# emiliofidalgo/liodom

Measured on AMD Instinct MI355X. Metric: scans/sec (64×1800 cloud, prev_frames=20) at 1 GPU; pose RMSE vs CPU ref, higher is better.
Workload: dtype f64

## Files before the change

liodom_amd/csrc/handle_plan.h:

```cpp
#pragma once
#include <algorithm>
#include <climits>
#include <cstdio>
#include <cstdlib>
#include <cstring>

#include "../../include/liodom_hip.h"
#include "liodom_sizes.h"

namespace liodom_dev {

struct HandleEnv {
  bool pipe_flags = true;
  bool map_rows = true;
  int hash_build = -1;
  int lds_cells_max = kLdsCellsMax;
  bool early_rebuild = true;
  bool safe_mode = false;
  int debug_clocks = 0;
  bool ring_split = true;
  bool ring_split_lb = true;
  int ring_pitch = 0;
  bool hash_incr = true;
  float rebuild_delta = 0.25f;
// ... 129 lines not shown
      config->n_streams < 1 || config->max_points < 1 || !(params->max_range > params->min_range)) {
    *error = "liodom_create: parameter out of range";
    return LIODOM_ERR_INVALID_ARG;
  }
  return LIODOM_OK;
}

inline int plan_handle(const liodom_params_t* params, const liodom_config_t* config, const HandleCaps& caps, const HandleEnv& env,
                       HandlePlan* out, const char** error) {
  using plan_detail::cdiv;
  using plan_detail::round_up;
  if (int rc = plan_check_params(params, config, error)) return rc;
  HandlePlan p;
  const int S = config->n_streams, H = params->scan_lines, P = (int)params->local_map_size;

  p.min_range = params->min_range; p.max_range = params->max_range;
  p.lidar_type = params->lidar_type; p.scan_lines = H;
  p.scan_regions = params->scan_regions; p.edges_per_region = params->edges_per_region;
  p.min_points_per_scan = (long long)params->min_points_per_scan;
  p.prev_frames = P;
  p.apply_on_ftol = config->lm_apply_step_on_ftol;
  p.rotation_mode = config->pose_rotation_mode != 0 ? 1 : 0;
  p.filter_local_map = (params->filter_local_map && !params->mapping) ? 1 : 0;
  p.vox_inv = 1.0f / 0.4f;
  p.n_streams = S;
  p.max_points = config->max_points;
  p.ring_cap = config->max_points;
  p.use_imu = params->use_imu ? 1 : 0;
  p.mapping = params->mapping ? 1 : 0;
  p.pose_log_cap = std::max(1, config->pose_log_capacity);
  p.pose_covariance = config->pose_covariance != 0;
  p.map_rows = env.map_rows;
  p.lds_cells_max = env.lds_cells_max;
  p.rebuild_delta = env.rebuild_delta;
  p.hb_slack_min = env.hb_slack; p.hb_new_room = env.hb_new_room;
  p.knn_save = env.knn_save;
  p.knn_exact_only = env.knn_exact_only ? 1 : 0;
  p.wait_ticks = (unsigned long long)(env.wait_ms * 1.0e5);
  p.lockstep = S >= 16;

  const long long slots = (long long)params->scan_regions * ((long long)params->edges_per_region + 1);
  if (slots > INT_MAX || ring_extract_lds_bytes((int)slots, params->scan_regions) > 160 * 1024) {
    *error = "pick lists (scan_regions * (edges_per_region + 1)) exceed 160 KiB of LDS";
    return LIODOM_ERR_CAPACITY;
  }
  p.slots_per_ring = (int)slots;
  p.ring_lds_bytes = ring_extract_lds_bytes(p.slots_per_ring, params->scan_regions);
  const int edges = H * p.slots_per_ring;
  p.edge_cap = (int)round_up(std::max(1, edges), 64);
  if (lm_lds_bytes(p.edge_cap) + 16384 > 160 * 1024) {
    *error = "liodom_create: edge capacity too large for the solve's LDS tile";
    return LIODOM_ERR_INVALID_ARG;
  }

  p.lds_hash_build = env.hash_build < 0 ? p.lockstep : env.hash_build != 0;

  p.use_flags = !p.lockstep && !env.serialised && env.pipe_flags;
  p.flag_gate = !(S == 1 && cdiv(cdiv(p.edge_cap, 8), 2) * 4 <= (long long)caps.cus * 12);

  {
    const int auto_g = S > 4 ? 1 : (edges >= 2048 ? kLmGroupsMax : (edges >= 512 ? 4 : 1));
    p.lm_groups = config->lm_workgroups == 0 ? auto_g : std::max(1, std::min(kLmGroupsMax, config->lm_workgroups));
  }

  p.early_rebuild = (!p.lds_hash_build && !p.filter_local_map && !params->mapping && S <= 4 && env.early_rebuild) ? 1 : 0;

  if (env.safe_mode) plan_enter_safe_mode(&p);

  p.recv_cap = p.mapping ? (config->recv_capacity > 0 ? config->recv_capacity : 262144) : 0;
  const long long map_cap = (long long)p.edge_cap * P + p.recv_cap;
  const long long pad = p.early_rebuild ? 8LL * p.edge_cap : 0;
  long long ts = 1024;
  while (ts < 2 * (map_cap + pad)) ts <<= 1;
  if (p.lds_hash_build && ts < kLdsSlots) ts = kLdsSlots;
  const long long used_cap = map_cap + pad;
  const long long ovf_base = map_cap + pad;
  long long sorted_cap = p.early_rebuild ? ovf_base + p.edge_cap : map_cap;
  const bool incr_sized = env.hash_incr && p.lockstep && p.lds_hash_build && !params->mapping && !params->filter_local_map && !p.early_rebuild;
  if (incr_sized) sorted_cap = 2 * map_cap + 65536 + (long long)(kHbPeriod - 1) * p.edge_cap;

  p.debug = config->debug_buffers & 1;
  if (caps.instrumented && env.debug_clocks != 0) {
    const int dc = env.debug_clocks;
    p.debug |= ((dc & (128 | 256)) ? (dc & 32) : 32) | (dc & (64 | 128)) | (dc & ~255);
  }
  const long long ring_id_stride = round_up((long long)config->max_points + 512, 256);
  p.tile_cap = (int)std::max(1LL, cdiv(config->max_points, kTilePts));
  p.split_pad = (int)round_up(p.tile_cap, 8);
  p.lb_hpad = (int)round_up(H, 64);
  p.ring_split_lb = p.lockstep && params->lidar_type == 0 && !p.safe_mode && env.ring_split_lb;
  const long long ring_pitch = env.ring_pitch ? env.ring_pitch : round_up(cdiv((long long)config->max_points * 9, (long long)H * 8), 8);

  if (ts > (1LL << 30) || map_cap > INT_MAX || used_cap > INT_MAX || sorted_cap > INT_MAX || ring_id_stride > INT_MAX || ring_pitch > INT_MAX) {
    *error = "liodom_create: capacities (window, received map, points per scan) exceed 32-bit sizes";
    return LIODOM_ERR_CAPACITY;
  }
  p.map_cap = (int)map_cap; p.table_size = (int)ts;
  p.used_cap = (int)used_cap; p.ovf_base = (int)ovf_base; p.sorted_cap = (int)sorted_cap;
  p.ring_id_stride = (size_t)ring_id_stride;
  p.ring_pitch = (int)ring_pitch;
  p.ring_stride = p.ring_split_lb ? std::max((size_t)config->max_points, (size_t)H * (size_t)p.ring_pitch) : (size_t)config->max_points;

  p.ring_split = env.ring_split && !p.safe_mode;
  if (p.ring_split) {
    long long budget = (long long)std::max(0, caps.ring_split_wgs_per_cu) * std::max(0, caps.cus) / 2;
    if (budget > 256) budget = 256;
    p.ring_split_max_wgs = (int)budget;
    if (p.tile_cap > p.ring_split_max_wgs) p.ring_split = false;
  }

  p.knn8 = p.lockstep && env.knn8;
  p.knn8_grid = (int)std::max(1LL, cdiv(cdiv(p.edge_cap, kKnn8Queries), kKnnGridDiv));
  p.hash_incr = (env.hash_incr && p.knn8 && p.lds_hash_build && !params->mapping && !params->filter_local_map && P > kHbPeriod &&
                 sorted_cap >= 2 * map_cap + (long long)(kHbPeriod - 1) * p.edge_cap) ? 1 : 0;
  p.hb_spill_base = p.sorted_cap - (kHbPeriod - 1) * p.edge_cap;
  p.knn_queries = p.lockstep ? 4 : 8;
  p.knn_partials = p.lockstep ? 0 : 1;
  p.knn_blocks = (int)round_up(cdiv(p.edge_cap, p.knn_queries), 4);
  p.knn_grid = (int)std::max(1LL, cdiv(p.knn_blocks, kKnnGridDiv));
  p.mask_stride = (int)round_up(p.knn_blocks, 128);

  p.ov_ok = env.knn_overlap != 0 && p.early_rebuild && S == 1 && p.knn_partials &&
            (env.knn_overlap == 2 || (long long)p.knn_grid * 4 * 3 <= (long long)caps.cus * 24);
  p.chain_ok = p.early_rebuild && S == 1 && p.knn_partials && !p.use_imu && (long long)p.knn_grid * 4 * 2 <= (long long)caps.cus * 24 &&
               env.knn_overlap != 0 && env.chain;
  p.speculate = (p.ov_ok || p.chain_ok) ? env.speculate : 0;
  p.spec_backoff = 16;
  p.spec_theta = env.spec_theta;

  *out = p;
  return LIODOM_OK;
}

struct OverlapModes { bool ov, chain; };
inline OverlapModes plan_overlap_modes(const HandlePlan& p, bool alone) {
  const bool base = p.early_rebuild && p.use_flags && alone;
  return {base && p.ov_ok, base && p.chain_ok && !p.flag_gate};
}

struct ModesRuntime {
  bool alone = true;
  bool streams_concurrent = true;
  int hb_stats[4] = {0, 0, 0, 0}, spec_stats[4] = {0, 0, 0, 0};
  unsigned int chain_count = 0, done0 = 0, done1 = 0;
  double replay_enqueue_us = 0.0, replay_wait_us = 0.0;
  int n_lagged = 0, n_readers = 0, n_hits = 0;
  long long subset_steps = 0;
};

inline void plan_format_modes(const HandlePlan& p, const ModesRuntime& r, char* buf, int cap) {
  const OverlapModes om = plan_overlap_modes(p, r.alone);
  snprintf(buf, (size_t)cap,
           "n_streams=%d early_rebuild=%d hash_build=%s pipe_flags=%d flag_gate=%d lm_groups=%d knn_instance=%d knn_queries=%d "
           "knn_grid=%d/%d knn8=%d hash_incr=%d hash_rebuilds=%d hash_appends=%d hash_appends_spilled=%d hash_points_spilled=%d knn_partials=%d knn_saved_bound=%d knn_exact_only=%d line_gate_kernel=%d filter_local_map=%d mapping=%d "
           "rotation_mode=%d table_size=%d sorted_cap=%d hb_spill_base=%d rebuild_delta=%.3f knn_overlap=%d streams_concurrent=%d safe_mode=%d ring_split=%d ring_split_max_wgs=%d ring_split_lb=%d chain=%d speculate=%d spec_early=%d/%d spec_unconfirmed=%d/%d chain_done=%u/%u/%u replay_enqueue_us=%.2f replay_wait_us=%.2f debug=%d",
           p.n_streams, p.early_rebuild, p.early_rebuild ? "streamed" : (p.lds_hash_build ? "lds" : "global"), p.use_flags ? 1 : 0,
           (p.use_flags && p.flag_gate) ? 1 : 0, p.lm_groups, p.lockstep ? 128 : 256, p.knn_queries, p.knn_grid,
           p.knn_blocks, p.knn8 ? 1 : 0, p.hash_incr, r.hb_stats[0], r.hb_stats[1], r.hb_stats[2], r.hb_stats[3], p.knn_partials,
           p.knn_save >= 2 ? 2 : (p.knn_save >= 1 ? 1 : 0), p.knn_exact_only, p.lockstep ? 1 : 0, p.filter_local_map, p.mapping,
           p.rotation_mode, p.table_size, p.sorted_cap, p.hb_spill_base, (double)p.rebuild_delta,
           (om.ov || om.chain) ? 1 : 0, r.streams_concurrent ? 1 : 0, p.safe_mode ? 1 : 0, p.ring_split ? 1 : 0, p.ring_split ? p.ring_split_max_wgs : 0, p.ring_split_lb ? 1 : 0,
           om.chain ? 1 : 0, p.speculate, r.spec_stats[0], r.spec_stats[2], r.spec_stats[1], r.spec_stats[3], r.chain_count, r.done0, r.done1,
           r.replay_enqueue_us, r.replay_wait_us, p.debug);
  auto tail = [&](size_t* room) { const size_t n = std::strlen(buf); *room = (size_t)cap - n; return buf + n; };
  size_t room = 0;
  if (p.pose_covariance) { char* t = tail(&room); snprintf(t, room, " pose_cov=1"); }
  if (r.n_lagged > 0) { char* t = tail(&room); snprintf(t, room, " mapper_lag=%d", r.n_lagged); }
// ... 7 lines not shown
```

liodom_amd/csrc/kernels_lm.h:

```cpp
constexpr int kLmWaves = kLmThreads / 64;


__device__ int lm_compact_bits(const DevView& v, int s, int outer_it, int E, int* idx ) {
  const int lane = threadIdx.x & 63;
  const int Q = v.knn_queries;
  const int nb = (E + Q - 1) / Q;
  const int nwords = (nb + 3) >> 2;
  const unsigned int* mw = reinterpret_cast<const unsigned int*>(v.corr_mask + ((size_t)s * 2 + outer_it) * v.mask_stride);
  int run = 0;
  for (int w0 = 0; w0 < nwords; w0 += 64) {
    const int w = w0 + lane;
    unsigned int word = (w < nwords) ? mw[w] : 0u;
    const int pop = __popc(word);
    const int incl = wave_incl_scan_i32(pop);
    int o = run + incl - pop;
    while (word) {
      const int b = __ffs(word) - 1;
      word &= word - 1u;
      const int bit = w * 32 + b;
      idx[o++] = (bit >> 3) * Q + (bit & 7);
    }
    run += readlane_i32(incl, 63);
  }
  return run;
// ... 238 lines not shown
  if (lane < 24) {
    const unsigned long long bits = (unsigned long long)__double_as_longlong(T[lane >> 1]);
    word = (lane & 1) ? (unsigned int)(bits >> 32) : (unsigned int)bits;
  }
  __hip_atomic_store((gu64*)(base + lane), ((unsigned long long)tag << 32) | word, __ATOMIC_RELAXED, __HIP_MEMORY_SCOPE_AGENT);
}

template <bool kList = false>
__global__ void k_imu_override(DevView v, int s0, int count) {
  const int i = blockIdx.x * blockDim.x + threadIdx.x;
  if (i >= count) return;
  const int s = stream_of_lane<kList>(v, s0, i);
  StreamState& st = v.state[s];
  if (!st.initialized) return;
  double odom[12], out[12], l2b[12], q[4];
#pragma unroll
  for (int k = 0; k < 12; k++) { odom[k] = st.odom[k]; l2b[k] = v.laser_to_base[k]; }
#pragma unroll
  for (int k = 0; k < 4; k++) q[k] = v.imu_q[(size_t)s * 4 + k];
  imu_override(odom, q, l2b, v.rotation_mode, out);
#pragma unroll
  for (int k = 0; k < 12; k++) st.odom[k] = out[k];
  quat_from_pose(out, v.rotation_mode, st.param_q);
  st.param_t[0] = out[3]; st.param_t[1] = out[7]; st.param_t[2] = out[11];
}

__device__ __forceinline__ void pose_cov_store(const DevView& v, int s, const StreamState& st, const LmState& lm, const double* acc, int nblocks, int tid) {
  const int j = tid - 64;
  if (j < 0 || j >= 21) return;
  PoseCovRaw* r = v.cov_raw + s;
  bool applied = lm.termination == LM_TERM_FUNC_TOL && lm.apply_on_ftol != 0;
  for (int k = 0; k < 4; k++) applied = applied && lm.q[k] == lm.cand_q[k];
  for (int k = 0; k < 3; k++) applied = applied && lm.t[k] == lm.cand_t[k];
  r->H[j] = applied ? acc[7 + j] : lm.H[j];
  if (j == 0) {
    r->scan_index = st.info.scan_index; r->n_res = nblocks; r->termination = lm.termination; r->has_solve = 1;
    r->cost = lm.cost;
  }
}

__device__ __forceinline__ void rebuild_beside_solve(const DevView& v, int s, StreamState& st, int eb, int outer_it, int block, int nblocks, unsigned int seq, int* sbase, int* sslot);

template <int kOuterIt, bool kChainMode, bool kList = false>
#ifndef LIODOM_LM_WAVES_PER_SIMD
#define LIODOM_LM_WAVES_PER_SIMD 1
#endif
__global__ __launch_bounds__(kLmThreads, LIODOM_LM_WAVES_PER_SIMD) void k_lm_solve(DevView v, int s0, int eb, unsigned int seq, unsigned int done_target) {
  constexpr int outer_it = kOuterIt;
  constexpr int chain = kChainMode ? 1 : 0;
  __shared__ double sh_pose2[2][12];
  __shared__ int sh_pi, sh_ci;
  __shared__ int sh_nmoved;
  __shared__ double sh_pred_s[20];
  __shared__ int sh_unapplied;
  __shared__ double sh_acc[kAccN];
  __shared__ LmState lm;
  __shared__ int sh_flag;
  __shared__ int sh_C;
  const int s = stream_of<kList>(v, s0, (int)blockIdx.y);
#if defined(LIODOM_CHAIN_PRIO)
  if (v.n_streams <= 4) __builtin_amdgcn_s_setprio(LIODOM_CHAIN_PRIO);
#endif
  const int G = v.lm_groups, gstride = G > 1 ? 8 : 1, bxl = (int)blockIdx.x;
  const bool is_solver = bxl < G * gstride && (bxl % gstride) == 0;
  const int g = is_solver ? bxl / gstride : G + (bxl < G * gstride ? bxl - (bxl / gstride + 1) : bxl - G);
  StreamState& st = v.state[s];
  __shared__ int sh_cnt[kMaxFrames + 1];
  OV_STAMP(v, bxl == 0 && threadIdx.x == 0, outer_it == 0 ? 0 : 3);
  if (seq && outer_it == 0 && bxl == 0 && threadIdx.x == 0) {
    typedef __attribute__((address_space(1))) unsigned int gu32;
    __hip_atomic_store((gu32*)(v.ov_flags + s), seq, __ATOMIC_RELAXED, __HIP_MEMORY_SCOPE_AGENT);
  }
  if (g >= G) {
    if (!v.early_rebuild || chain) return;
    __shared__ int sh_slot[kMaxFrames];
    rebuild_beside_solve(v, s, st, eb, outer_it, g - G, (int)gridDim.x - G, seq, sh_cnt, sh_slot);
    return;
  }
  __shared__ double sh_wsum[kLmWaves][32];
  __shared__ double sh_red[16][32];
  __shared__ double sh_x0[8];
  __shared__ double sh_prev[12];
  __shared__ int sh_fc;
  if (threadIdx.x < 4) sh_x0[threadIdx.x] = st.param_q[threadIdx.x];
  else if (threadIdx.x < 7) sh_x0[threadIdx.x] = st.param_t[threadIdx.x - 4];
  else if (threadIdx.x >= 64 && threadIdx.x < 76) sh_prev[threadIdx.x - 64] = st.prev_odom[threadIdx.x - 64];
  else if (threadIdx.x == 76) sh_fc = st.frame_count;
  __shared__ int sh_spec_at;
  if (threadIdx.x == 77) sh_spec_at = st.spec_eval[outer_it];
  __shared__ int sh_redo;
  if (threadIdx.x == 78) sh_redo = st.spec_redo[outer_it == 0 ? 1 : 0];
  extern __shared__ __attribute__((aligned(16))) int sh_idx[];
  const int tid = threadIdx.x;
  const bool prep = tid < kLmCtl;
  bool dead = false;
  if (chain && outer_it == 0) dead = !chain_wait_count(v.knn_done0 + s, done_target, &st.status);
  if (chain && outer_it == 0 && sh_redo) __builtin_amdgcn_fence(__ATOMIC_ACQUIRE, "agent");
  int E_in;
  if (chain && outer_it == 0) {
    typedef __attribute__((address_space(1))) unsigned int gu32;
    E_in = (int)__hip_atomic_load((gu32*)(v.edge_cnt + eb * 32 + s), __ATOMIC_RELAXED, __HIP_MEMORY_SCOPE_AGENT);
  } else {
    E_in = st.n_edges_buf[eb];
  }
  if (outer_it == 0 && tid == 0 && g == 0) {
    st.info.n_edges = E_in;
    st.info.map_points = st.n_search;
    for (int k = 0; k < 2; k++) {
      st.info.lm[k].iterations = 0; st.info.lm[k].accepted = 0; st.info.lm[k].termination = LM_TERM_NO_RESIDUALS;
      st.info.lm[k].pad = 0; st.info.lm[k].initial_cost = 0.0; st.info.lm[k].final_cost = 0.0;
    }
  }
  if (!st.initialized) {
    if (outer_it == 1 && g == 0) {
      if (seq) ov_wait_knn_done(v, s, seq, &st.status);
      if (tid == 0) st.append_raw = 1;
      __shared__ double sh_T0[12];
      if (tid < 12) sh_T0[tid] = st.odom[tid];
      __syncthreads();
      finalize_scan(v, s, st, sh_cnt, eb, true, 0, 0, sh_T0, 1, true, sh_prev, sh_fc);
      if (tid == 0) st.initialized = 1;
      if (v.cov_raw && tid == 64) {
        PoseCovRaw* r = v.cov_raw + s;
        r->scan_index = st.info.scan_index; r->n_res = 0; r->termination = st.info.lm[1].termination; r->has_solve = 0; r->cost = st.info.lm[1].final_cost;
      }
    }
    return;
  }
  bool clr_pending = outer_it == 1 && g == 0 && prep && !v.early_rebuild;
  auto clear_hash_slots = [&]() {
    hash_clear_used(v, s, st.n_used_tab[0], tid, kLmCtl);
    clr_pending = false;
  };
  const bool dbgb = (s == 0) && (g == 0) && (tid == kLmCtl) && (outer_it == 1);
  const bool dbge = (s == 0) && (g == 0) && (tid == 0) && (outer_it == 1);
  DBG_STAMP(v, dbgb, 2, 0);
  const int E = E_in;
  int nblocks = st.info.matches[outer_it];
  __shared__ int sh_nmatch;
  __shared__ double sh_scale[8];
  const unsigned int epoch0 = ((unsigned int)(st.scan_counter + 1) << 6) | ((unsigned int)outer_it << 5);
  unsigned int n_eval = 0;
  bool xch_local = false;
  LmCache cache;
  int c_lo = 0, c_hi = 0;
  int dbg_it = 0;
  auto evaluate = [&](const double* pose) {
    lm_eval(v, s, outer_it, eb, c_lo, c_hi, sh_idx, pose, &sh_wsum[0][0], cache);
    if (tid >= kLmCtl) {
      const int lane = tid - kLmCtl;
      if (G > 1) {
        const double x = lm_wave_total(&sh_wsum[0][0], c_hi - c_lo, lane >> 1);
        DBG_STAMP(v, dbgb && dbg_it < 4, 2, 12 + dbg_it);
        xch_local = lm_exchange(v, s, g, G, epoch0 | ++n_eval, x, sh_acc, &st.status, xch_local, lane);
      } else {
        if (lane < kAccN) sh_acc[lane] = lm_wave_total(&sh_wsum[0][0], c_hi - c_lo, lane);
        ++n_eval;
      }
      asm volatile("s_waitcnt lgkmcnt(0)" ::: "memory");
      __builtin_amdgcn_wave_barrier();
    }
  };
  auto my_share = [&](int C) {
    const int chunk = (C + G - 1) / G;
    c_lo = g * chunk < C ? g * chunk : C;
    c_hi = (g + 1) * chunk < C ? (g + 1) * chunk : C;
  };
  if (seq && outer_it == 1) { if (chain) dead = !chain_wait_count(v.knn_done0 + 32 + s, done_target, &st.status) || dead; else ov_wait_knn_done(v, s, seq, &st.status); }
  if (seq && outer_it == 1) { __syncthreads(); if (sh_redo) __builtin_amdgcn_fence(__ATOMIC_ACQUIRE, "agent"); }
  OV_STAMP(v, g == 0 && tid == 0 && outer_it == 1, 4);
  OV_STAMP(v, g == 0 && tid == 0 && outer_it == 0, 18);
  if (v.knn_partials) {
    const int Q = v.knn_queries;
    const int nb = (E + Q - 1) / Q;
    const double* part = v.knn_part + ((size_t)s * 2 + outer_it) * v.knn_blocks * 32;
    constexpr int kRC = kLmThreads / 32;
    const int i = tid & 31, r0 = tid >> 5;
    double x0 = 0.0, x1 = 0.0;
    if (i <= kAccN) {
      const int nb_cap = v.knn_blocks;
      for (int rb = r0; rb < (dead ? 0 : (rb == r0 ? nb_cap : nb)); rb += 16 * kRC) {
        double xs[16];
#pragma unroll
        for (int u = 0; u < 16; u++) { const int r = rb + kRC * u; xs[u] = (r < nb_cap) ? part[(size_t)r * 32 + i] : 0.0; }
#pragma unroll
        for (int u = 0; u < 16; u++) { const int r = rb + kRC * u; if (r >= nb) xs[u] = 0.0; }
#pragma unroll
        for (int u = 0; u < 16; u += 2) { x0 += xs[u]; x1 += xs[u + 1]; }
      }
    }
    sh_red[r0][i] = x0 + x1;
    __syncthreads();
    if (tid <= kAccN) {
      double x = 0.0;
#pragma unroll
      for (int r = 0; r < kRC; r++) x += sh_red[r][tid];
      if (tid < kAccN) sh_acc[tid] = x;
      else { sh_nmatch = (int)x; if (g == 0) st.info.matches[outer_it] = (int)x; }
    }
    __syncthreads();
    nblocks = sh_nmatch;
  } else {
    __syncthreads();
    if (prep) {
      const int C = lm_compact_bits(v, s, outer_it, E, sh_idx);
      if (tid == 0) sh_C = C;
    } else if (tid == kLmCtl) {
      iso_from_qt(sh_x0, sh_x0 + 4, sh_pose2[0]);
    }
    __syncthreads();
    my_share(sh_C);
    lm_cache_load(v, s, outer_it, eb, c_lo, c_hi, sh_idx, cache);
    evaluate(sh_pose2[0]);
  }
  DBG_STAMP(v, dbgb, 2, 2);
  int pi = 0, ci = -1, nmoved = 0;
  const unsigned int n_eval0 = n_eval;
  const bool spec_ok = v.speculate != 0 && v.speculate != 5 && v.speculate != 7 && g == 0 && seq != 0u && outer_it == 0;
  const bool spec_ok1 = v.speculate != 0 && v.speculate != 4 && v.speculate != 6 && g == 0 && chain != 0 && outer_it == 1 && v.early_rebuild && v.pred_xch != nullptr;
  const bool spec_forced = v.speculate == 2 || v.speculate == 6 || v.speculate == 7;
  bool spec_done = false;
  int spec_moves = -1;
  for (int step = 0;; step++) {
    if (step == 0 && tid > kLmCtl && tid <= kLmCtl + 6) {
      const int j = tid - kLmCtl - 1;
      sh_scale[j] = 1.0 / (1.0 + sqrt(sh_acc[7 + h_idx(j, j)]));
    }
    if (step == 0) __builtin_amdgcn_wave_barrier();
    if (tid == kLmCtl) {
      const int acc_before = step == 0 ? 0 : lm.accepted;
      const int f = step == 0 ? lm_begin(lm, sh_x0, sh_x0 + 4, sh_acc, nblocks, v.apply_on_ftol, sh_scale) : lm_update(lm, sh_acc);
      sh_flag = f;
      bool moved = step > 0 && lm.accepted != acc_before;
      if (step > 0 && !moved && f != LM_NEED_EVAL && lm.termination == LM_TERM_FUNC_TOL) {
        moved = true;
        for (int k = 0; k < 4; k++) moved = moved && lm.q[k] == lm.cand_q[k];
        for (int k = 0; k < 3; k++) moved = moved && lm.t[k] == lm.cand_t[k];
      }
      if (moved) { ci = pi; pi ^= 1; nmoved++; }
      if (f == LM_NEED_EVAL) iso_from_qt(lm.cand_q, lm.cand_t, sh_pose2[pi]);
      sh_pi = pi; sh_ci = ci; sh_nmoved = nmoved; sh_unapplied = (step > 0 && !moved) ? 1 : 0;
      if (step == 0) DBG_STAMP(v, dbgb, 2, 23);
    } else if (!prep) {
    } else if (step == 0 && v.knn_partials) {
      DBG_STAMP(v, dbge, 2, 24);
      const int C = dead ? 0 : lm_compact_bits(v, s, outer_it, E, sh_idx);
      if (tid == 0) sh_C = C;
      DBG_STAMP(v, dbge, 2, 25);
      my_share(C);
      lm_cache_load(v, s, outer_it, eb, c_lo, c_hi, sh_idx, cache);
    } else if (clr_pending) {
      clear_hash_slots();
    }
    __syncthreads();
    if (step == 0) { if (v.knn_partials && !prep) my_share(sh_C); DBG_STAMP(v, dbgb, 2, 3); }
    else { DBG_STAMP(v, dbgb && dbg_it < 5, 2, 5 + 2 * dbg_it); dbg_it++; }
    if (sh_flag != LM_NEED_EVAL) break;
    if ((spec_ok || spec_ok1) && !spec_done && sh_ci >= 0 &&
        (spec_forced || (!spec_forced && sh_spec_at == 0 && lm.model_cost_change <= v.spec_theta * 1e-6 * lm.cost))) {
      if (spec_ok) {
        ov_publish_pose(v, s, sh_pose2[sh_ci], &lm.q[0], seq, tid, 1);
        OV_STAMP(v, tid == 0, 19);
      } else if (tid >= kLmCtl) {
        const int l = tid - kLmCtl;
        if (l < 25) publish_final_pose(v, s, sh_pose2[sh_ci], 0, (unsigned int)sh_fc + 1u, l, 0);
        if (l == 0) predict_next(sh_pose2[sh_ci], sh_prev, v.rotation_mode, sh_pred_s);
        asm volatile("s_waitcnt lgkmcnt(0)" ::: "memory");
        __builtin_amdgcn_wave_barrier();
        pred_publish(v, s, sh_pred_s, (unsigned int)sh_fc + 1u, l, 64, 1);
        OV_STAMP(v, l == 0, 22);
      }
      if ((kInstrument && (v.debug & 64)) && tid == 0) atomicAdd(&v.dbg_clk[270], 1ull);
      spec_done = true;
      spec_moves = sh_nmoved;
    }
    const double* pose_c = sh_pose2[sh_pi];
    evaluate(pose_c);
    DBG_STAMP(v, dbgb && dbg_it < 5, 2, 4 + 2 * dbg_it);
  }
  if (clr_pending) clear_hash_slots();
  DBG_STAMP(v, dbgb, 2, 20);
  if ((kInstrument && (v.debug & 32)) && dbgb) v.dbg_clk[2 * 32 + 27] = (xch_local ? 100ull : 0ull) + 10ull * xcc_id() + (unsigned long long)n_eval;
  if (g != 0) return;
  __shared__ double sh_ov[20];
  __shared__ liodom_lm_trace_t sh_trace;
  {
    if (tid == kLmCtl) {
      sh_trace.iterations = lm.iter; sh_trace.accepted = lm.accepted; sh_trace.termination = lm.termination; sh_trace.pad = 0;
      sh_trace.initial_cost = lm.initial_cost; sh_trace.final_cost = lm.cost;
    }
    const int cif = sh_ci;
    if (cif >= 0) {
      if (tid < 12) sh_ov[tid] = sh_pose2[cif][tid];
      else if (tid >= 64 && tid < 71) sh_ov[12 + tid - 64] = (&lm.q[0])[tid - 64];
    } else if (tid == kLmCtl) {
      double q[4], t[3], T[12];
      for (int k = 0; k < 4; k++) q[k] = lm.q[k];
      for (int k = 0; k < 3; k++) t[k] = lm.t[k];
      iso_from_qt(q, t, T);
      for (int k = 0; k < 12; k++) sh_ov[k] = T[k];
      for (int k = 0; k < 4; k++) sh_ov[12 + k] = q[k];
      for (int k = 0; k < 3; k++) sh_ov[16 + k] = t[k];
    }
  }
  __syncthreads();
  if (outer_it == 0) {
    if (seq) { ov_publish_pose(v, s, sh_ov, sh_ov + 12, seq, tid, spec_done ? 2 : 3); OV_STAMP(v, tid == 0, 1); }
  } else if (v.early_rebuild && tid < 50) {
    if (tid >= 25 || !spec_done) publish_final_pose(v, s, sh_ov, 0, (unsigned int)sh_fc + 1u, tid % 25, tid / 25);
  }
  if (tid == kLmCtl) {
    if (outer_it == 0) {
      for (int k = 0; k < 4; k++) st.param_q[k] = sh_ov[12 + k];
      for (int k = 0; k < 3; k++) st.param_t[k] = sh_ov[16 + k];
// ... 18 lines not shown
```

liodom_amd/csrc/liodom_kernels.h:

```cpp
#pragma once
#include <hip/hip_runtime.h>

#include <cstddef>

#include "../../include/liodom_hip.h"
#include "liodom_math.h"
#include "liodom_sizes.h"
#include "stream_state_format.h"
#include "wave_ops.h"

namespace liodom_dev {

#ifndef LIODOM_CHAIN_PRIO
#define LIODOM_CHAIN_PRIO 2
#endif
constexpr int kWave = 64;
constexpr uint64_t kEmptyKey = 0xFFFFFFFFFFFFFFFFull;
constexpr int kLmEvalThreads = kLmThreads;
constexpr int kLmCtl = kLmThreads - 64;
constexpr int kKnnGroup = 32;
constexpr int kEdgeBufX = 3;
constexpr int kOvReplicas = 8;
constexpr int kOvGranules = 38;
constexpr int kPredGranules = 38;
// ... 140 lines not shown
  double* knn_part;
  unsigned char* corr_mask;
  int mask_stride;
  int knn_partials;
  int knn_queries;
  unsigned int* cell_pad;
  int used_cap;
  int sorted_cap;
  int ovf_base;
  float rebuild_delta;
  int hb_spill_base;
  int hb_slack_min, hb_new_room;
  int hash_incr;
  unsigned int* cell_cap;
  int* knn8_cnt;
  int* knn8_list;
  float4* knn_nn;
  unsigned int* pipe_flags;
  unsigned long long* pose_xch;
  unsigned int* redo_sync;
  int early_rebuild;
  int knn_grid;
  float4* knn_save_q;
  int2* knn_save_pos;
  float* knn_save_g;
  int knn_exact_only;
  int knn_blocks;
  unsigned long long* lm_xch;
  unsigned int* ov_flags;
  double spec_theta;
  int spec_backoff;
  int speculate;
  unsigned long long* pose_xch0;
  unsigned int* knn_done;
  float4* edges_keep;
  unsigned int* pub_counter;
  unsigned int* edge_cnt;
  unsigned int* knn_done0;
  unsigned long long* pred_xch;
  float4* host_edges;
  int4* host_edges_meta;
  unsigned int* host_edges_hdr;
  unsigned long long* dbg_clk;
  unsigned int* dbg_q;
  PoseCovRaw* cov_raw;
  liodom_pose_cov_t* cov_log;
  HostCov* cov_host;
};

__device__ __forceinline__ bool filter_active(const DevView& v, const StreamState& st) {
  return v.filter_local_map != 0 && st.n_frames == v.prev_frames;
}

typedef const __attribute__((address_space(4))) int* stream_list_ptr;
__device__ __forceinline__ stream_list_ptr stream_list(const DevView& v, int s0) {
  return (stream_list_ptr)(reinterpret_cast<const int*>(v.pipe_flags) + kStreamListBase + (size_t)(-s0 - 1) * (size_t)v.n_streams);
}
template <bool kList>
__device__ __forceinline__ int stream_of(const DevView& v, int s0, int row) {
  if constexpr (!kList) return s0 + row;
  else return stream_list(v, s0)[__builtin_amdgcn_readfirstlane(row)];
}
template <bool kList>
__device__ __forceinline__ int stream_of_lane(const DevView& v, int s0, int row) {
  if constexpr (!kList) return s0 + row;
  else return stream_list(v, s0)[row];
}
template <bool kList>
__device__ __forceinline__ int scan_row_of(int s0, int row, int s) { (void)s0; return kList ? s : row; }
struct StreamListChunk { int s[kStreamListChunk]; };
__global__ __launch_bounds__(kStreamListChunk) void k_put_list(DevView v, int list, int first, int count, StreamListChunk c) {
  int* dst = reinterpret_cast<int*>(v.pipe_flags) + kStreamListBase + (size_t)list * (size_t)v.n_streams + first;
  if ((int)threadIdx.x < count) dst[threadIdx.x] = c.s[threadIdx.x];
}

__device__ __forceinline__ int lane_id() { return threadIdx.x & (kWave - 1); }
#if defined(LIODOM_INSTRUMENT)
constexpr bool kInstrument = true;
#else
constexpr bool kInstrument = false;
#endif
#define DBG_STAMP(v, cond, k, i) do { if (kInstrument && ((v).debug & 32) && (cond)) (v).dbg_clk[(k) * 32 + (i)] = wall_clock64(); } while (0)
#define OV_STAMP(v, cond, i) do { if (kInstrument && ((v).debug & 128) && (cond)) (v).dbg_clk[448 + (i)] = wall_clock64(); } while (0)
#define DBG_QSTAMP(i) do { if (kInstrument && (kInstrument && (v.debug & 32)) && s == 0 && hl == 0 && e < E) v.dbg_q[((size_t)outer_it * v.edge_cap + e) * 12 + (i)] = (unsigned int)(wall_clock64() - t_blk); } while (0)

__device__ __forceinline__ void xcd_remap(int& bx, int& by) {
  const int nbx = (int)gridDim.x, nby = (int)gridDim.y;
  if (nby < 8 || (nby & 7)) return;
  const int lin = bx + nbx * by;
  const int xcd = lin & 7, slot = lin >> 3;
  by = (slot / nbx) * 8 + xcd;
  bx = slot - (slot / nbx) * nbx;
}

__device__ __forceinline__ unsigned long long pack_cell(int cx, int cy, int cz) {
  const unsigned long long m = 0x1FFFFFull;
  return ((unsigned long long)(cx & m) << 42) | ((unsigned long long)(cy & m) << 21) |
         (unsigned long long)(cz & m);
}
__device__ __forceinline__ unsigned int hash_cell(unsigned long long k, unsigned int mask) {
  const unsigned int x = (unsigned int)(k >> 42), y = (unsigned int)(k >> 21) & 0x1FFFFFu, z = (unsigned int)k & 0x1FFFFFu;
  unsigned int h = (x * 73856093u) ^ (y * 19349663u) ^ (z * 83492791u);
  h ^= h >> 16; h *= 0x85ebca6bu; h ^= h >> 13; h *= 0xc2b2ae35u; h ^= h >> 16;
  return h & mask;
}

__device__ unsigned long long g_wait_ticks = 5000000ull;
__device__ __forceinline__ bool wait_expired(unsigned int spins, unsigned long long& t0) {
  if ((spins & 31u) != 0u) return false;
  const unsigned long long now = wall_clock64();
  if (t0 == 0ull) { t0 = now; return false; }
  return now - t0 > g_wait_ticks;
}

#if defined(LIODOM_INJECT_DELAY)
__device__ unsigned int g_inject_seed = 0u;
__device__ __forceinline__ void inject_delay(unsigned int site) {
  const unsigned int seed = g_inject_seed;
  if (!seed) return;
  unsigned int h = seed ^ (site * 0x9E3779B1u) ^ ((unsigned int)blockIdx.x * 0x85EBCA6Bu) ^ ((unsigned int)blockIdx.y * 0xC2B2AE35u) ^ (unsigned int)wall_clock64();
  h ^= h >> 16; h *= 0x7FEB352Du; h ^= h >> 15; h *= 0x846CA68Bu; h ^= h >> 16;
  h = __builtin_amdgcn_readfirstlane(h);
  if ((h & 3u) != 0u) return;
  const unsigned int n = (h >> 2) % 48u;
  for (unsigned int i = 0; i < n; i++) __builtin_amdgcn_s_sleep(16);
}
#define INJECT_DELAY(site) inject_delay(site)
#else
#define INJECT_DELAY(site) do { } while (0)
#endif

#include "kernels_extract.h"
#include "kernels_sync.h"
#include "kernels_compact.h"
#include "kernels_knn.h"
#include "kernels_knn8.h"
#include "kernels_lm.h"
#include "kernels_rebuild.h"
#include "kernels_filter.h"
#include "kernels_cov.h"
#include "kernels_state.h"
#include "kernels_polar.h"
#include "kernels_mapper.h"

}
```

liodom_amd/csrc/liodom_math.h:

```cpp
#pragma once
#include <cfloat>
#include <cmath>
#include <cstdint>

#if defined(__HIPCC__)
#define LD_HD __host__ __device__ __forceinline__
#define LD_UNROLL _Pragma("unroll")
#define LD_FP_CONTRACT_FAST _Pragma("clang fp contract(fast)")
#else
#define LD_HD inline
#define LD_UNROLL
#define LD_FP_CONTRACT_FAST
#endif
#if defined(__HIP_DEVICE_COMPILE__)
#define LD_RSQRT(x) rsqrt(x)
#else
#define LD_RSQRT(x) (1.0 / sqrt(x))
#endif

namespace liodom_dev {

constexpr int kJacobiSweeps = 8;
constexpr int kLmMaxIterations = 4;
constexpr double kHuberA = 0.2;
// ... 723 lines not shown
      AS[i * 6 + j] = s;
    }
  }
  LD_UNROLL
  for (int i = 0; i < 6; i++) {
    LD_UNROLL
    for (int j = 0; j < 6; j++) {
      double s = 0.0;
      LD_UNROLL
      for (int k = 0; k < 6; k++) s += AS[i * 6 + k] * A[j * 6 + k];
      out36[i * 6 + j] = s;
    }
  }
}

LD_HD double norm7(const double* q, const double* t) {
  LD_FP_CONTRACT_FAST
  return sqrt(q[0] * q[0] + q[1] * q[1] + q[2] * q[2] + q[3] * q[3] + t[0] * t[0] + t[1] * t[1] + t[2] * t[2]);
}

LD_HD int lm_propose(LmState& st) {
  LD_FP_CONTRACT_FAST
  while (true) {
    if (st.iter >= kLmMaxIterations) { st.termination = LM_TERM_MAX_ITER; return LM_DONE; }
    if (st.radius < 1e-32) { st.termination = LM_TERM_RADIUS; return LM_DONE; }
    st.iter++;
    double sc[6], gs[6];
    LD_UNROLL
    for (int i = 0; i < 6; i++) { sc[i] = st.scale[i]; gs[i] = sc[i] * st.g[i]; }
    double A[21];
    LD_UNROLL
    for (int i = 0; i < 6; i++) {
      LD_UNROLL
      for (int j = 0; j <= i; j++) A[lt_idx(i, j)] = sc[i] * sc[j] * st.H[h_idx(j, i)];
    }
    if (!st.reuse_diagonal) {
      LD_UNROLL
      for (int j = 0; j < 6; j++) {
        double d = A[lt_idx(j, j)];
        if (d < 1e-6) d = 1e-6;
        if (d > 1e32) d = 1e32;
        st.diag[j] = d;
      }
    }
    const double inv_radius = 1.0 / st.radius;
    LD_UNROLL
    for (int j = 0; j < 6; j++) A[lt_idx(j, j)] += st.diag[j] * inv_radius;
    double y[6];
    const bool ok = chol_solve6_packed(A, gs, y);
    st.reuse_diagonal = 1;
    double mcc = 0.0;
    double step[6];
    if (ok) {
      double sg = 0.0, shs = 0.0;
      LD_UNROLL
      for (int i = 0; i < 6; i++) step[i] = -y[i];
      LD_UNROLL
      for (int i = 0; i < 6; i++) {
        sg += step[i] * gs[i];
        double row = 0.0;
        LD_UNROLL
        for (int j = 0; j < i; j++) row += (sc[i] * sc[j] * st.H[h_idx(j, i)]) * step[j];
        shs += step[i] * (2.0 * row + (sc[i] * sc[i] * st.H[h_idx(i, i)]) * step[i]);
      }
      mcc = -sg - 0.5 * shs;
    }
    if (!ok || !(mcc > 0.0)) {
      if (++st.invalid_run >= 5) { st.termination = LM_TERM_INVALID_STEPS; return LM_DONE; }
      st.radius = st.radius * 0.5;
      continue;
    }
    st.invalid_run = 0;
    st.model_cost_change = mcc;
    double delta[6];
    LD_UNROLL
    for (int j = 0; j < 6; j++) delta[j] = step[j] * sc[j];
    quat_plus(st.q, delta, st.cand_q);
    LD_UNROLL
    for (int k = 0; k < 3; k++) st.cand_t[k] = st.t[k] + delta[3 + k];
    return LM_NEED_EVAL;
  }
}

LD_HD int lm_begin(LmState& st, const double* q0, const double* t0, const double* acc,
                   int n_blocks, int apply_on_ftol, const double* pre_scale = nullptr) {
  LD_UNROLL
  for (int k = 0; k < 4; k++) st.q[k] = st.cand_q[k] = q0[k];
  LD_UNROLL
  for (int k = 0; k < 3; k++) st.t[k] = st.cand_t[k] = t0[k];
  st.iter = 0; st.accepted = 0; st.invalid_run = 0; st.termination = LM_TERM_MAX_ITER;
  st.apply_on_ftol = apply_on_ftol;
  st.cost = 0.0; st.initial_cost = 0.0; st.model_cost_change = 0.0;
  st.radius = 1e4; st.decrease_factor = 2.0; st.reuse_diagonal = 0;
  LD_UNROLL
  for (int j = 0; j < 6; j++) { st.scale[j] = 1.0; st.diag[j] = 0.0; st.g[j] = 0.0; }
  LD_UNROLL
  for (int j = 0; j < 21; j++) st.H[j] = 0.0;
  st.x_norm = norm7(st.q, st.t);
  if (n_blocks == 0) { st.termination = LM_TERM_NO_RESIDUALS; return LM_DONE; }
  if (acc[28] != 0.0) { st.termination = LM_TERM_EVAL_FAILURE; return LM_DONE; }
  st.cost = acc[0]; st.initial_cost = acc[0];
  double gmax = 0.0;
  LD_UNROLL
  for (int j = 0; j < 6; j++) { st.g[j] = acc[1 + j]; const double ag = fabs(st.g[j]); if (ag > gmax) gmax = ag; }
  LD_UNROLL
  for (int j = 0; j < 21; j++) st.H[j] = acc[7 + j];
  LD_UNROLL
  for (int j = 0; j < 6; j++) st.scale[j] = pre_scale ? pre_scale[j] : 1.0 / (1.0 + sqrt(st.H[h_idx(j, j)]));
  if (gmax <= 1e-10) { st.termination = LM_TERM_GRAD_TOL; return LM_DONE; }
  return lm_propose(st);
}

LD_HD int lm_update(LmState& st, const double* acc) {
  LD_FP_CONTRACT_FAST
  const double cand_cost = (acc[28] != 0.0) ? DBL_MAX : acc[0];
  double dq[4], dt[3];
  LD_UNROLL
  for (int k = 0; k < 4; k++) dq[k] = st.q[k] - st.cand_q[k];
  LD_UNROLL
  for (int k = 0; k < 3; k++) dt[k] = st.t[k] - st.cand_t[k];
  const double step_sq = dq[0] * dq[0] + dq[1] * dq[1] + dq[2] * dq[2] + dq[3] * dq[3] + dt[0] * dt[0] + dt[1] * dt[1] + dt[2] * dt[2];
  const double ptol = 1e-8 * (st.x_norm + 1e-8);
  const double ptol_sq = ptol * ptol;
  bool ptol_hit = step_sq <= ptol_sq * (1.0 - 1e-12);
  if (!ptol_hit && step_sq <= ptol_sq * (1.0 + 1e-12)) ptol_hit = sqrt(step_sq) <= ptol;
  if (ptol_hit) { st.termination = LM_TERM_PARAM_TOL; return LM_DONE; }
  const double cost_change = st.cost - cand_cost;
  if (fabs(cost_change) <= 1e-6 * st.cost) {
    st.termination = LM_TERM_FUNC_TOL;
    if (st.apply_on_ftol && cost_change > 0.0) {
      LD_UNROLL
      for (int k = 0; k < 4; k++) st.q[k] = st.cand_q[k];
      LD_UNROLL
      for (int k = 0; k < 3; k++) st.t[k] = st.cand_t[k];
      st.cost = cand_cost;
    }
    return LM_DONE;
  }
  const double rel = cost_change / st.model_cost_change;
  if (rel > 1e-3) {
    LD_UNROLL
    for (int k = 0; k < 4; k++) st.q[k] = st.cand_q[k];
    LD_UNROLL
    for (int k = 0; k < 3; k++) st.t[k] = st.cand_t[k];
    st.x_norm = norm7(st.q, st.t);
    st.cost = cand_cost;
    double gmax = 0.0;
    LD_UNROLL
    for (int j = 0; j < 6; j++) { st.g[j] = acc[1 + j]; const double ag = fabs(st.g[j]); if (ag > gmax) gmax = ag; }
    LD_UNROLL
    for (int j = 0; j < 21; j++) st.H[j] = acc[7 + j];
    st.accepted++;
    const double c = 2.0 * rel - 1.0;
    double f = 1.0 - c * c * c;
    if (f < 1.0 / 3.0) f = 1.0 / 3.0;
    st.radius = st.radius / f;
    if (st.radius > 1e16) st.radius = 1e16;
    st.decrease_factor = 2.0;
    st.reuse_diagonal = 0;
    if (gmax <= 1e-10) { st.termination = LM_TERM_GRAD_TOL; return LM_DONE; }
  } else {
    st.radius = st.radius / st.decrease_factor;
    st.decrease_factor *= 2.0;
    st.reuse_diagonal = 1;
  }
  return lm_propose(st);
}

LD_HD void pg_quat_mul(const double* a, const double* b, double* o) {
  o[3] = a[3] * b[3] - a[0] * b[0] - a[1] * b[1] - a[2] * b[2];
  o[0] = a[3] * b[0] + a[0] * b[3] + a[1] * b[2] - a[2] * b[1];
  o[1] = a[3] * b[1] + a[1] * b[3] + a[2] * b[0] - a[0] * b[2];
  o[2] = a[3] * b[2] + a[2] * b[3] + a[0] * b[1] - a[1] * b[0];
}
LD_HD void pg_rot3(const double* q, double* R ) {
  const double x = q[0], y = q[1], z = q[2], w = q[3];
  const double tx = 2 * x, ty = 2 * y, tz = 2 * z;
  const double twx = tx * w, twy = ty * w, twz = tz * w;
  const double txx = tx * x, txy = ty * x, txz = tz * x;
  const double tyy = ty * y, tyz = tz * y, tzz = tz * z;
  R[0] = 1 - (tyy + tzz); R[1] = txy - twz;       R[2] = txz + twy;
  R[3] = txy + twz;       R[4] = 1 - (txx + tzz); R[5] = tyz - twx;
  R[6] = txz - twy;       R[7] = tyz + twx;       R[8] = 1 - (txx + tyy);
}
LD_HD void graph_edge_error(const double* Xi, const double* Xj, const double* Z, double* e, double* A, double* B) {
  double Ri[9], Rz[9];
  pg_rot3(Xi, Ri);
  pg_rot3(Z, Rz);
  const double u[3] = {Xj[4] - Xi[4], Xj[5] - Xi[5], Xj[6] - Xi[6]};
  double m[3];
  LD_UNROLL
  for (int r = 0; r < 3; r++) m[r] = (Ri[r] * u[0] + Ri[3 + r] * u[1] + Ri[6 + r] * u[2]) - Z[4 + r];
  const double ci[4] = {-Xi[0], -Xi[1], -Xi[2], Xi[3]}, cz[4] = {-Z[0], -Z[1], -Z[2], Z[3]};
// ... 150 lines not shown
```

liodom_amd/csrc/liodom_sizes.h:

```cpp
#pragma once
#include <cstddef>

#if defined(__HIPCC__)
#define LS_HD __host__ __device__ __forceinline__
#else
#define LS_HD inline
#endif

namespace liodom_dev {

#ifndef LIODOM_LM_THREADS
#define LIODOM_LM_THREADS 256
#endif
constexpr int kLmThreads = LIODOM_LM_THREADS;
#ifndef LIODOM_LM_GROUPS_MAX
#define LIODOM_LM_GROUPS_MAX 8
#endif
constexpr int kLmGroupsMax = LIODOM_LM_GROUPS_MAX;
constexpr int kMaxFrames = 256;
constexpr int kEdgeBufs = 4;
constexpr int kEdgePipeBufs = 3;

constexpr int kTilePts = 2048;
constexpr int kTileChunks = kTilePts / 64;
constexpr int kTileThreads = 512;
constexpr int kRowThreads = 512;

LS_HD int ring_scatter_stride(int H) { return H | 1; }
LS_HD size_t ring_scatter_stage_bytes(int H) {
  const int Hp = ring_scatter_stride(H);
  const size_t a = (size_t)kTileChunks * Hp * 8 + (size_t)((kTileChunks * Hp * 2 + 15) & ~15);
  const size_t b = (size_t)kTilePts * 24;
  return a > b ? a : b;
}
LS_HD size_t ring_scatter_lds_bytes(int H) {
  return ring_scatter_stage_bytes(H) + (size_t)(2 * H + 2 * 16) * 4;
}
LS_HD size_t ring_split_lb_lds_bytes(int H) {
  return ring_scatter_stage_bytes(H) + (size_t)(3 * H + 16) * 4;
}

constexpr int kExLPR = 16;
constexpr int kExIPL = 16;
constexpr int kExIPLBig = 24;
constexpr int kGapBitsCap = 16384;
constexpr int kExMaxRegions = 64;

LS_HD int ring_extract_threads(int regions) {
  const int waves = (regions + 3) / 4;
  return 64 * (waves < 1 ? 1 : (waves > 16 ? 16 : waves));
}
LS_HD size_t ring_extract_lds_bytes(int slots, int regions) {
  size_t b = (size_t)(kGapBitsCap / 32 + 4) * 4;
  b += (size_t)slots * 4;
  b += (size_t)((slots + 15) / 16 * 16);
  b += (size_t)regions * 4 + 2 * kExMaxRegions * 4 + 64;
  return (b + 15) / 16 * 16;
}

constexpr int kCompactBlocks = 8;

constexpr int kKnnGridDiv = 2;
constexpr int kG8 = 8;
#ifndef LIODOM_KNN8_THREADS
#define LIODOM_KNN8_THREADS 256
#endif
constexpr int kKnn8Threads = LIODOM_KNN8_THREADS;
constexpr int kKnn8Queries = kKnn8Threads / kG8;
constexpr int kKnn8ExactBlocks = 4;

LS_HD size_t lm_lds_bytes(int edge_cap) {
  return (size_t)((edge_cap + 3) & ~3) * sizeof(int);
}

constexpr int kRebuildAuxBlocks = 8;
constexpr int kRebuildAllocBlocks = 32;
#ifndef LIODOM_REBFIN_THREADS
#define LIODOM_REBFIN_THREADS LIODOM_LM_THREADS
#endif
constexpr int kRebFinThreads = LIODOM_REBFIN_THREADS;

constexpr int kBuildThreads = 1024;
constexpr int kLdsSlots = 8192;
constexpr int kLdsCellsMax = 6144;
LS_HD size_t hash_build_lds_bytes() { return (size_t)kLdsSlots * 16 + 64; }
#ifndef LIODOM_HB_PERIOD
#define LIODOM_HB_PERIOD 4
#endif
constexpr int kHbPeriod = LIODOM_HB_PERIOD;
constexpr int kHbNewRoom = 96;
constexpr int kHbSlackMin = 32;

constexpr int kMapRowsThreads = 256;

}
```

Baseline: 14510.

## Split LM begin into state/sum phases and widen guarded partial-sum reduction

```diff
diff --git a/liodom_amd/csrc/handle_plan.h b/liodom_amd/csrc/handle_plan.h
--- a/liodom_amd/csrc/handle_plan.h
+++ b/liodom_amd/csrc/handle_plan.h
@@ -235,7 +235,7 @@
   p.debug = config->debug_buffers & 1;
   if (caps.instrumented && env.debug_clocks != 0) {
     const int dc = env.debug_clocks;
-    p.debug |= ((dc & (128 | 256)) ? (dc & 32) : 32) | (dc & (64 | 128)) | (dc & ~255);
+    p.debug |= ((dc & (128 | 256 | 512)) ? (dc & 32) : 32) | (dc & (64 | 128)) | (dc & ~255);
   }
   const long long ring_id_stride = round_up((long long)config->max_points + 512, 256);
   p.tile_cap = (int)std::max(1LL, cdiv(config->max_points, kTilePts));
diff --git a/liodom_amd/csrc/kernels_lm.h b/liodom_amd/csrc/kernels_lm.h
--- a/liodom_amd/csrc/kernels_lm.h
+++ b/liodom_amd/csrc/kernels_lm.h
@@ -344,9 +344,10 @@
   __shared__ double sh_x0[8];
   __shared__ double sh_prev[12];
   __shared__ int sh_fc;
-  if (threadIdx.x < 4) sh_x0[threadIdx.x] = st.param_q[threadIdx.x];
-  else if (threadIdx.x < 7) sh_x0[threadIdx.x] = st.param_t[threadIdx.x - 4];
-  else if (threadIdx.x >= 64 && threadIdx.x < 76) sh_prev[threadIdx.x - 64] = st.prev_odom[threadIdx.x - 64];
+  const int ctl_lane = (int)threadIdx.x - kLmCtl;
+  if (ctl_lane >= 0 && ctl_lane < 4) sh_x0[ctl_lane] = st.param_q[ctl_lane];
+  else if (ctl_lane >= 4 && ctl_lane < 7) sh_x0[ctl_lane] = st.param_t[ctl_lane - 4];
+  if (threadIdx.x >= 64 && threadIdx.x < 76) sh_prev[threadIdx.x - 64] = st.prev_odom[threadIdx.x - 64];
   else if (threadIdx.x == 76) sh_fc = st.frame_count;
   __shared__ int sh_spec_at;
   if (threadIdx.x == 77) sh_spec_at = st.spec_eval[outer_it];
@@ -355,6 +356,11 @@
   extern __shared__ __attribute__((aligned(16))) int sh_idx[];
   const int tid = threadIdx.x;
   const bool prep = tid < kLmCtl;
+  if (v.knn_partials && ctl_lane >= 0) {
+    asm volatile("s_waitcnt lgkmcnt(0)" ::: "memory");
+    __builtin_amdgcn_wave_barrier();
+    if (ctl_lane == 0) lm_begin_state(lm, sh_x0, sh_x0 + 4, v.apply_on_ftol);
+  }
   bool dead = false;
   if (chain && outer_it == 0) dead = !chain_wait_count(v.knn_done0 + s, done_target, &st.status);
   if (chain && outer_it == 0 && sh_redo) __builtin_amdgcn_fence(__ATOMIC_ACQUIRE, "agent");
@@ -403,6 +409,7 @@
   __shared__ double sh_scale[8];
   const unsigned int epoch0 = ((unsigned int)(st.scan_counter + 1) << 6) | ((unsigned int)outer_it << 5);
   unsigned int n_eval = 0;
+  const int hscan = (kInstrument && (v.debug & 512)) ? st.scan_counter : 0;
   bool xch_local = false;
   LmCache cache;
   int c_lo = 0, c_hi = 0;
@@ -432,6 +439,7 @@
   if (seq && outer_it == 1) { __syncthreads(); if (sh_redo) __builtin_amdgcn_fence(__ATOMIC_ACQUIRE, "agent"); }
   OV_STAMP(v, g == 0 && tid == 0 && outer_it == 1, 4);
   OV_STAMP(v, g == 0 && tid == 0 && outer_it == 0, 18);
+  HANDIN_STAMP(v, g == 0 && tid == 0, hscan, outer_it, 0);
   if (v.knn_partials) {
     const int Q = v.knn_queries;
     const int nb = (E + Q - 1) / Q;
@@ -440,18 +448,29 @@
     const int i = tid & 31, r0 = tid >> 5;
     double x0 = 0.0, x1 = 0.0;
     if (i <= kAccN) {
-      const int nb_cap = v.knn_blocks;
-      for (int rb = r0; rb < (dead ? 0 : (rb == r0 ? nb_cap : nb)); rb += 16 * kRC) {
-        double xs[16];
-#pragma unroll
-        for (int u = 0; u < 16; u++) { const int r = rb + kRC * u; xs[u] = (r < nb_cap) ? part[(size_t)r * 32 + i] : 0.0; }
-#pragma unroll
-        for (int u = 0; u < 16; u++) { const int r = rb + kRC * u; if (r >= nb) xs[u] = 0.0; }
-#pragma unroll
-        for (int u = 0; u < 16; u += 2) { x0 += xs[u]; x1 += xs[u + 1]; }
+      constexpr bool late_count = chain && outer_it == 0;
+      const int nb_tab = v.knn_blocks, nb_lim = nb < nb_tab ? nb : nb_tab;
+      for (int rb = r0; rb < (dead ? 0 : (rb == r0 ? (late_count ? nb_tab : nb_lim) : nb)); rb += kLmPartRows * kRC) {
+        double xs[kLmPartRows];
+#pragma unroll
+        for (int c = 0; c < kLmPartRows / kLmPartRowsEarly; c++) {
+          const int cap = (late_count && c == 0 && rb == r0) ? nb_tab : nb_lim;
+          if (rb + kRC * kLmPartRowsEarly * c < cap) {
+#pragma unroll
+            for (int u = kLmPartRowsEarly * c; u < kLmPartRowsEarly * (c + 1); u++) { const int r = rb + kRC * u; xs[u] = part[(size_t)(r < cap ? r : 0) * 32 + i]; }
+          } else {
+#pragma unroll
+            for (int u = kLmPartRowsEarly * c; u < kLmPartRowsEarly * (c + 1); u++) xs[u] = 0.0;
+          }
+        }
+#pragma unroll
+        for (int u = 0; u < kLmPartRows; u++) { const int r = rb + kRC * u; if (r >= nb_lim) xs[u] = 0.0; }
+#pragma unroll
+        for (int u = 0; u < kLmPartRows; u += 2) { x0 += xs[u]; x1 += xs[u + 1]; }
       }
     }
     sh_red[r0][i] = x0 + x1;
+    HANDIN_STAMP(v, g == 0 && tid == kLmCtl, hscan, outer_it, 1);
     __syncthreads();
     if (tid <= kAccN) {
       double x = 0.0;
@@ -469,6 +488,7 @@
       if (tid == 0) sh_C = C;
     } else if (tid == kLmCtl) {
       iso_from_qt(sh_x0, sh_x0 + 4, sh_pose2[0]);
+      lm_begin_state(lm, sh_x0, sh_x0 + 4, v.apply_on_ftol);
     }
     __syncthreads();
     my_share(sh_C);
@@ -491,7 +511,9 @@
     if (step == 0) __builtin_amdgcn_wave_barrier();
     if (tid == kLmCtl) {
       const int acc_before = step == 0 ? 0 : lm.accepted;
-      const int f = step == 0 ? lm_begin(lm, sh_x0, sh_x0 + 4, sh_acc, nblocks, v.apply_on_ftol, sh_scale) : lm_update(lm, sh_acc);
+      HANDIN_STAMP(v, g == 0 && step == 0, hscan, outer_it, 2);
+      const int f = step == 0 ? lm_begin_sums(lm, sh_acc, nblocks, sh_scale) : lm_update(lm, sh_acc);
+      HANDIN_STAMP(v, g == 0 && step == 0, hscan, outer_it, 3);
       sh_flag = f;
       bool moved = step > 0 && lm.accepted != acc_before;
       if (step > 0 && !moved && f != LM_NEED_EVAL && lm.termination == LM_TERM_FUNC_TOL) {
diff --git a/liodom_amd/csrc/liodom_kernels.h b/liodom_amd/csrc/liodom_kernels.h
--- a/liodom_amd/csrc/liodom_kernels.h
+++ b/liodom_amd/csrc/liodom_kernels.h
@@ -246,6 +246,7 @@
 #endif
 #define DBG_STAMP(v, cond, k, i) do { if (kInstrument && ((v).debug & 32) && (cond)) (v).dbg_clk[(k) * 32 + (i)] = wall_clock64(); } while (0)
 #define OV_STAMP(v, cond, i) do { if (kInstrument && ((v).debug & 128) && (cond)) (v).dbg_clk[448 + (i)] = wall_clock64(); } while (0)
+#define HANDIN_STAMP(v, cond, scan, it, i) do { if (kInstrument && ((v).debug & 512) && (cond)) (v).dbg_clk[((scan) & 63) * 8 + (it) * 4 + (i)] = wall_clock64(); } while (0)
 #define DBG_QSTAMP(i) do { if (kInstrument && (kInstrument && (v.debug & 32)) && s == 0 && hl == 0 && e < E) v.dbg_q[((size_t)outer_it * v.edge_cap + e) * 12 + (i)] = (unsigned int)(wall_clock64() - t_blk); } while (0)
 
 __device__ __forceinline__ void xcd_remap(int& bx, int& by) {
diff --git a/liodom_amd/csrc/liodom_math.h b/liodom_amd/csrc/liodom_math.h
--- a/liodom_amd/csrc/liodom_math.h
+++ b/liodom_amd/csrc/liodom_math.h
@@ -829,8 +829,7 @@
   }
 }
 
-LD_HD int lm_begin(LmState& st, const double* q0, const double* t0, const double* acc,
-                   int n_blocks, int apply_on_ftol, const double* pre_scale = nullptr) {
+LD_HD void lm_begin_state(LmState& st, const double* q0, const double* t0, int apply_on_ftol) {
   LD_UNROLL
   for (int k = 0; k < 4; k++) st.q[k] = st.cand_q[k] = q0[k];
   LD_UNROLL
@@ -844,6 +843,8 @@
   LD_UNROLL
   for (int j = 0; j < 21; j++) st.H[j] = 0.0;
   st.x_norm = norm7(st.q, st.t);
+}
+LD_HD int lm_begin_sums(LmState& st, const double* acc, int n_blocks, const double* pre_scale = nullptr) {
   if (n_blocks == 0) { st.termination = LM_TERM_NO_RESIDUALS; return LM_DONE; }
   if (acc[28] != 0.0) { st.termination = LM_TERM_EVAL_FAILURE; return LM_DONE; }
   st.cost = acc[0]; st.initial_cost = acc[0];
@@ -856,6 +857,11 @@
   for (int j = 0; j < 6; j++) st.scale[j] = pre_scale ? pre_scale[j] : 1.0 / (1.0 + sqrt(st.H[h_idx(j, j)]));
   if (gmax <= 1e-10) { st.termination = LM_TERM_GRAD_TOL; return LM_DONE; }
   return lm_propose(st);
+}
+LD_HD int lm_begin(LmState& st, const double* q0, const double* t0, const double* acc,
+                   int n_blocks, int apply_on_ftol, const double* pre_scale = nullptr) {
+  lm_begin_state(st, q0, t0, apply_on_ftol);
+  return lm_begin_sums(st, acc, n_blocks, pre_scale);
 }
 
 LD_HD int lm_update(LmState& st, const double* acc) {
diff --git a/liodom_amd/csrc/liodom_sizes.h b/liodom_amd/csrc/liodom_sizes.h
--- a/liodom_amd/csrc/liodom_sizes.h
+++ b/liodom_amd/csrc/liodom_sizes.h
@@ -13,6 +13,9 @@
 #define LIODOM_LM_THREADS 256
 #endif
 constexpr int kLmThreads = LIODOM_LM_THREADS;
+constexpr int kLmPartRows = 48;
+constexpr int kLmPartRowsEarly = 16;
+static_assert(kLmPartRows % kLmPartRowsEarly == 0 && kLmPartRowsEarly % 2 == 0, "whole groups of an even number of rows");
 #ifndef LIODOM_LM_GROUPS_MAX
 #define LIODOM_LM_GROUPS_MAX 8
 #endif
```

After: 13200. -9.0%, worse.
